# rcanut/nhwcodec

Hardware: AMD Instinct MI355X
Metric: encode Mpixels/s (512x512 RGB batch) (higher is better)
Workload: dtype int16

## Files before the change

nhwcodec_amd/csrc/nhw_tail_wave.h:

```cpp
#include <type_traits>
#ifndef NHW_TAIL_WAVE_H
#define NHW_TAIL_WAVE_H

#include "nhw_tail_dev.h"

namespace nhw {

struct M4 { uint64_t w[4]; };
DEV M4 operator&(M4 a, M4 b) { return M4{ { a.w[0] & b.w[0], a.w[1] & b.w[1], a.w[2] & b.w[2], a.w[3] & b.w[3] } }; }
DEV M4 operator|(M4 a, M4 b) { return M4{ { a.w[0] | b.w[0], a.w[1] | b.w[1], a.w[2] | b.w[2], a.w[3] | b.w[3] } }; }
DEV M4 operator~(M4 a) { return M4{ { ~a.w[0], ~a.w[1], ~a.w[2], ~a.w[3] } }; }
DEV M4 m4_zero() { return M4{ { 0, 0, 0, 0 } }; }
DEV M4 up1(M4 a) { return M4{ { a.w[0] << 1, (a.w[1] << 1) | (a.w[0] >> 63), (a.w[2] << 1) | (a.w[1] >> 63), (a.w[3] << 1) | (a.w[2] >> 63) } }; }
DEV M4 dn1(M4 a) { return M4{ { (a.w[0] >> 1) | (a.w[1] << 63), (a.w[1] >> 1) | (a.w[2] << 63), (a.w[2] >> 1) | (a.w[3] << 63), a.w[3] >> 1 } }; }
DEV M4 dn2(M4 a) { return M4{ { (a.w[0] >> 2) | (a.w[1] << 62), (a.w[1] >> 2) | (a.w[2] << 62), (a.w[2] >> 2) | (a.w[3] << 62), a.w[3] >> 2 } }; }
DEV M4 dn3(M4 a) { return M4{ { (a.w[0] >> 3) | (a.w[1] << 61), (a.w[1] >> 3) | (a.w[2] << 61), (a.w[2] >> 3) | (a.w[3] << 61), a.w[3] >> 3 } }; }
DEV uint64_t low_bits(int n) { return n <= 0 ? 0ull : (n >= 64 ? ~0ull : ((1ull << n) - 1)); }
DEV M4 col_range(int lo, int hi)
{
	M4 r;
	r.w[0] = low_bits(hi + 1) & ~low_bits(lo);
	r.w[1] = low_bits(hi + 1 - 64) & ~low_bits(lo - 64);
	r.w[2] = low_bits(hi + 1 - 128) & ~low_bits(lo - 128);
	r.w[3] = low_bits(hi + 1 - 192) & ~low_bits(lo - 192);
	return r;
}
#define TB(m, k) ((int)__builtin_amdgcn_inverse_ballot_w64((m).w[k]))
#define BALLOT4(m, arr, expr) do { { const int x = arr[0]; (m).w[0] = __ballot(expr); } { const int x = arr[1]; (m).w[1] = __ballot(expr); } \
	{ const int x = arr[2]; (m).w[2] = __ballot(expr); } { const int x = arr[3]; (m).w[3] = __ballot(expr); } } while (0)

template <int N> DEV unsigned bs_up(unsigned b, int lane, unsigned in0 = 0)
{
	const unsigned seam = (((unsigned)__builtin_amdgcn_readlane((int)b, 63) << 1) | in0) & ((1u << N) - 1);
	(void)lane;
	return (unsigned)__builtin_amdgcn_update_dpp((int)seam, (int)b, 0x138 , 0xF, 0xF, false);
}
DEV unsigned bs_dn(unsigned b, int lane)
{
	const unsigned seam = (unsigned)__builtin_amdgcn_readlane((int)b, 0) >> 1;
	(void)lane;
	return (unsigned)__builtin_amdgcn_update_dpp((int)seam, (int)b, 0x130 , 0xF, 0xF, false);
}
#define BS_PREDK(b, arr, k0, expr) do { (b) = 0; for (int k_ = (k0); k_ < 4; k_++) { const int x = (arr)[k_]; (b) |= ((expr) ? 1u : 0u) << k_; } } while (0)
#define BS_PRED(b, arr, n, expr) do { (b) = 0; for (int k_ = 0; k_ < (n); k_++) { const int x = (arr)[k_]; (b) |= ((expr) ? 1u : 0u) << k_; } } while (0)
DEV M4 bs_ballot4(unsigned b) { return M4{ { __ballot(b & 1), __ballot(b & 2), __ballot(b & 4), __ballot(b & 8) } }; }
DEV unsigned bs_from4(M4 m) { unsigned b = 0; for (int k = 0; k < 4; k++) b |= (unsigned)__builtin_amdgcn_inverse_ballot_w64(m.w[k]) << k; return b; }

DEV M4 alt_runs(M4 f)
{
	const uint64_t even = 0x5555555555555555ull;
	const M4 pf = up1(f);
	uint64_t sum[4];
	unsigned carry = 0;
	for (int k = 0; k < 4; k++) {
		const uint64_t se = f.w[k] & ~pf.w[k] & even;
		const uint64_t t = f.w[k] + se;
		const unsigned c1 = t < se;
		sum[k] = t + carry;
		carry = c1 | (sum[k] < t);
	}
	M4 r;
	for (int k = 0; k < 4; k++) {
		const uint64_t re = f.w[k] & ~sum[k];
		r.w[k] = (re & even) | (f.w[k] & ~re & ~even);
	}
	return r;
}

DEV int right_of(const int *v, int k, int nk, int d, int lane)
{
	const int a = __shfl(v[k], (lane + d) & 63);
	const int b = k + 1 < nk ? __shfl(v[k + 1], (lane + d) & 63) : 0;
	return lane + d < 64 ? a : b;
}

DEV int ll2_round(int v) { return (v > 0 && v < 256) ? (v & 0xFFFE) : v; }

DEV void ll2_load_row(const int16_t *p, int r, int lane, int *v, M4 *tag, int q, int part, M4 *starts = nullptr, int ps = W )
{
	if (starts) *starts = m4_zero();
	if (r >= H / 2) { v[0] = v[1] = v[2] = 0; *tag = m4_zero(); return; }
	for (int k = 0; k < 3; k++) v[k] = p[r * ps + lane + 64 * k];
	M4 t = m4_zero();
	if (q > 17) {
		int v4[4] = { v[0], v[1], v[2], 0 };
		M4 o, d3;
		BALLOT4(o, v4, x & 1);
		int far[4];
		for (int k = 0; k < 2; k++) far[k] = right_of(v, k, 3, 3, lane);
		d3.w[0] = __ballot(iabs(v[0] - far[0]) > 1); d3.w[1] = __ballot(iabs(v[1] - far[1]) > 1); d3.w[2] = d3.w[3] = 0;
		const M4 f = o & dn1(o) & dn2(o) & dn3(o) & d3 & col_range(0, H / 2 - 4);
		unsigned __int128 m = ((unsigned __int128)f.w[1] << 64) | f.w[0], tg = 0;
		const unsigned __int128 pat = part ? 5 : 15;
		unsigned __int128 st = 0;
		while (m) {
			const uint64_t lo = (uint64_t)m;
			const int j = lo ? __builtin_ctzll(lo) : 64 + __builtin_ctzll((uint64_t)(m >> 64));
			tg |= pat << j; st |= (unsigned __int128)1 << j;
			m &= ~((unsigned __int128)15 << j);
		}
		t.w[0] = (uint64_t)tg; t.w[1] = (uint64_t)(tg >> 64);
		if (starts) { starts->w[0] = (uint64_t)st; starts->w[1] = (uint64_t)(st >> 64); }
	}
	*tag = t;
}

DEV void wave_ll2_verbatim(Ctx *c, int lane)
{
	if (c->defer_verbatim) return;
	__threadfence_block();
	const int nm = c->m->ll_mem_len;
	for (int i = lane; i < nm; i += 64) {
		const int idx = c->ll_mem[i], pos = ((idx >> 7) << 9) + (idx & 127);
		c->jpeg[pos] = c->proc[pos];
	}
}

DEV void wave_ll2(Ctx *c, int part, int lane, bool keep_p, const int16_t *src, int ss )
{
	int16_t *p = c->proc, *jp = c->jpeg;
	const int q = c->q;
	int v0[3], v1[3], v2[3], v3[3];
	M4 t0, t1, t2, t3;
	ll2_load_row(src, 0, lane, v0, &t0, q, part, nullptr, ss);
	ll2_load_row(src, 1, lane, v1, &t1, q, part, nullptr, ss);
	ll2_load_row(src, 2, lane, v2, &t2, q, part, nullptr, ss);
	ll2_load_row(src, 3, lane, v3, &t3, q, part, nullptr, ss);
	const M4 ll = col_range(0, H / 2 - 1);
	for (int r = 0; r < H / 2; r++) {
		int vn[3]; M4 tn;
		ll2_load_row(src, r + 4, lane, vn, &tn, q, part, nullptr, ss);
		if (q > 17) {
			int a0[4] = { v0[0], v0[1], v0[2], 0 }, a1[4] = { v1[0], v1[1], v1[2], 0 }, a2[4] = { v2[0], v2[1], 0, 0 }, a3[4] = { v3[0], v3[1], 0, 0 };
			M4 o, o1, o2, o3, d2;
			BALLOT4(o, a0, x & 1); BALLOT4(o1, a1, x & 1); BALLOT4(o2, a2, x & 1); BALLOT4(o3, a3, x & 1);
			const int f0 = right_of(v0, 0, 3, 2, lane), f1 = right_of(v0, 1, 3, 2, lane);
			d2.w[0] = __ballot(iabs(v0[0] - f0) > 1); d2.w[1] = __ballot(iabs(v0[1] - f1) > 1); d2.w[2] = d2.w[3] = 0;
			d2 = d2 | dn2(t0);
			const M4 cond1 = o & dn1(o) & col_range(1, H / 2 - 1);
			const M4 hbr = cond1 & dn2(o) & col_range(0, H / 2 - 3);
			const M4 skip = part ? up1(t0) : m4_zero();
			const M4 act = ll & ~t0 & ~skip;
			const M4 fired = alt_runs(hbr & d2 & act);
			const M4 bumped = up1(fired);
			M4 vf = m4_zero();
			if (r <= H / 2 - 2) vf = cond1 & ~hbr & o1 & dn1(o1) & ~dn2(o1);
			if (r >= 1 && r <= H / 2 - 4) vf = vf | (~cond1 & o & o1 & dn1(o1) & o2 & ~o3);
			vf = vf & act & ~bumped & ~t1;
			for (int k = 0; k < 2; k++) { v0[k] += TB(bumped, k); v1[k] += TB(vf, k); }
		}
		for (int k = 0; k < 2; k++) {
			const int at = r * W + lane + 64 * k;
			if (keep_p || !part) p[at] = (int16_t)v0[k];
			jp[at] = (int16_t)(TB(t0, k) ? v0[k] : ll2_round(v0[k]));
		}
		for (int k = 0; k < 3; k++) { v0[k] = v1[k]; v1[k] = v2[k]; v2[k] = v3[k]; v3[k] = vn[k]; }
		t0 = t1; t1 = t2; t2 = t3; t3 = tn;
	}
	if (!part) wave_ll2_verbatim(c, lane);
	__threadfence_block();
}

DEV void wave_emit_ll2(Ctx *c, int lane, bool sim)
{
	int16_t *p = c->proc, *jp = c->jpeg;
	const int q = c->q;
	int v0[3], v1[3], v2[3], v3[3];
	M4 t0, t1, t2, t3, s0, s1, s2, s3;
	ll2_load_row(p, 0, lane, v0, &t0, q, 0, &s0);
	ll2_load_row(p, 1, lane, v1, &t1, q, 0, &s1);
	ll2_load_row(p, 2, lane, v2, &t2, q, 0, &s2);
	ll2_load_row(p, 3, lane, v3, &t3, q, 0, &s3);
	const M4 ll = col_range(0, H / 2 - 1);
	int n4 = 0, e = 0, carry = 0;
	for (int r = 0; r < H / 2; r++) {
		int vn[3]; M4 tn, sn;
		ll2_load_row(p, r + 4, lane, vn, &tn, q, 0, &sn);
		if (q > 17) {
			int a0[4] = { v0[0], v0[1], v0[2], 0 }, a1[4] = { v1[0], v1[1], v1[2], 0 }, a2[4] = { v2[0], v2[1], 0, 0 }, a3[4] = { v3[0], v3[1], 0, 0 };
			M4 o, o1, o2, o3, d2;
			BALLOT4(o, a0, x & 1); BALLOT4(o1, a1, x & 1); BALLOT4(o2, a2, x & 1); BALLOT4(o3, a3, x & 1);
			const int f0 = right_of(v0, 0, 3, 2, lane), f1 = right_of(v0, 1, 3, 2, lane);
			d2.w[0] = __ballot(iabs(v0[0] - f0) > 1); d2.w[1] = __ballot(iabs(v0[1] - f1) > 1); d2.w[2] = d2.w[3] = 0;
			d2 = d2 | dn2(t0);
			const M4 cond1 = o & dn1(o) & col_range(1, H / 2 - 1);
			const M4 hbr = cond1 & dn2(o) & col_range(0, H / 2 - 3);
			const M4 act = ll & ~t0;
			const M4 bumped = up1(alt_runs(hbr & d2 & act));
			M4 vf = m4_zero();
			if (r <= H / 2 - 2) vf = cond1 & ~hbr & o1 & dn1(o1) & ~dn2(o1);
			if (r >= 1 && r <= H / 2 - 4) vf = vf | (~cond1 & o & o1 & dn1(o1) & o2 & ~o3);
			vf = vf & act & ~bumped & ~t1;
			for (int k = 0; k < 2; k++) v1[k] += TB(vf, k);
			for (int k = 0; k < 2; k++) v0[k] += TB(bumped, k);
		}
		uint64_t x[2], g[2];
		int byte[2];
		for (int k = 0; k < 2; k++) {
			const int s = v0[k];
			x[k] = __ballot(s > 255 || s < 0);
			byte[k] = s > 255 ? 255 : (s < 0 ? 0 : s);
		}
		if (r == 0) x[0] &= ~1ull;
		g[0] = ~x[0]; g[1] = ~x[1];
		for (int k = 0; k < 2; k++) {
			const int col = lane + 64 * k, a = r * (H / 2) + col;
			const bool exc = (x[k] >> lane) & 1;
			const uint64_t hi = k ? (g[1] & low_bits(lane)) : 0, lo = k ? g[0] : (g[0] & low_bits(lane));
			const int src = hi ? 64 + 63 - __builtin_clzll(hi) : (lo ? 63 - __builtin_clzll(lo) : -1);
			const int b0 = __shfl(byte[0], src & 63), b1 = __shfl(byte[1], src & 63);
			const int prev = src < 0 ? carry : (((src >> 6) ? b1 : b0) & 254);
			if (exc) {
				const int s = v0[k], mag = s > 255 ? s - 255 : -s;
				const int rank = __popcll(x[0] & (k ? ~0ull : low_bits(lane))) + (k ? __popcll(x[1] & low_bits(lane)) : 0);
				uint8_t *ex = c->exw + e + 3 * rank;
				ex[0] = (uint8_t)r; ex[1] = (uint8_t)(col + (s > 255 ? 128 : 0)); ex[2] = (uint8_t)(mag > 255 ? 255 : mag);
				c->ll_bytes[a] = (uint8_t)prev; c->ll_full[a] = (uint8_t)prev;
			} else { c->ll_full[a] = (uint8_t)byte[k]; c->ll_bytes[a] = (uint8_t)(byte[k] & 254); }
			p[r * W + col] = (int16_t)(sim ? v0[k] : 0);
			if (sim) jp[r * W + col] = (int16_t)(TB(t0, k) ? v0[k] : ll2_round(v0[k]));
		}
		e += 3 * (__popcll(x[0]) + __popcll(x[1]));
		if (g[1]) carry = __shfl(byte[1], 63 - __builtin_clzll(g[1])) & 254;
		else if (g[0]) carry = __shfl(byte[0], 63 - __builtin_clzll(g[0])) & 254;
		if (q > 17) {
			const int cnt = __popcll(s0.w[0]) + __popcll(s0.w[1]);
			if (!cnt) { if (lane == 0) c->res4[n4] = 128; n4++; }
			else {
				for (int k = 0; k < 2; k++)
					if ((s0.w[k] >> lane) & 1) {
						const int rank = __popcll(s0.w[0] & (k ? ~0ull : low_bits(lane))) + (k ? __popcll(s0.w[1] & low_bits(lane)) : 0);
						c->res4[n4 + rank] = (uint8_t)(lane + 64 * k + 1 + (rank == cnt - 1 ? 128 : 0));
					}
				n4 += cnt;
			}
		}
		for (int k = 0; k < 3; k++) { v0[k] = v1[k]; v1[k] = v2[k]; v2[k] = v3[k]; v3[k] = vn[k]; }
		t0 = t1; t1 = t2; t2 = t3; t3 = tn;
		s0 = s1; s1 = s2; s2 = s3; s3 = sn;
	}
	if (lane == 0) { c->m->res4_len = q > 17 ? n4 : 0; c->m->exw_len = e; }
}

DEV void det_load_row(const int16_t *p, int r, int lane, int *v, int ps = W)
{
	if (r >= H) { v[0] = v[1] = v[2] = v[3] = 0; return; }
	const bool top = r < H / 2;
	v[0] = top ? 0 : p[r * ps + lane];
	v[1] = top ? 0 : p[r * ps + lane + 64];
	v[2] = p[r * ps + lane + 128];
	v[3] = p[r * ps + lane + 192];
}

DEV unsigned bs_range(int lo, int hi, int lane)
{
	unsigned b = 0;
	for (int k = 0; k < 4; k++) { const int col = lane + 64 * k; b |= (col >= lo && col <= hi ? 1u : 0u) << k; }
	return b;
}

#define DQ_LIM 512
#define DQ_MARK0 (2 * DQ_LIM + 1)
#define DQ_WORDS (DQ_MARK0 + 126)
enum : unsigned { DQ_E8 = 1u << 16, DQ_E7 = 1u << 17, DQ_EM7 = 1u << 18, DQ_DC = 1u << 19, DQ_AC = 1u << 20, DQ_BIG = 1u << 21, DQ_CODE = 1u << 22, DQ_K2 = 1u << 23, DQ_K1 = 1u << 24, DQ_PRP = 1u << 25, DQ_PRN = 1u << 26 };
DEV int dq_index(int x)
{
	const int d = x - 15300;
	const int cl = x < -DQ_LIM ? -DQ_LIM : x > DQ_LIM ? DQ_LIM : x;
	return ((unsigned)d <= 500u && !(d & 3)) ? DQ_MARK0 + (d >> 2) : cl + DQ_LIM;
}
DEV unsigned dq_entry(int i)
{
	if (i >= DQ_MARK0) {
		const int d = 4 * (i - DQ_MARK0);
		if (d % 100) return DQ_BIG;
		const int x = 15300 + d;
		const int v = (x == 15300 || x == 15500) ? 5 : (x == 15400 || x == 15600) ? -5 : x == 15700 ? 6 : -6;
		return (unsigned)(uint16_t)(int16_t)v | DQ_CODE | (x <= 15400 ? DQ_K2 : DQ_K1) | (x == 15700 ? DQ_PRP : 0u) | (x == 15800 ? DQ_PRN : 0u);
	}
	const int x = i - DQ_LIM;
	if (x >= DQ_LIM || x <= -DQ_LIM) return DQ_BIG;
	int a = x;
	if (a < 0) { a = -a; if ((a & 7) < 7) a &= 0xFFF8; a = -a; }
	unsigned e = (unsigned)(uint16_t)(int16_t)dequant_value(a);
	if (x == 8) e |= DQ_E8;
	if (x == 7) e |= DQ_E7;
	if (x == -7) e |= DQ_EM7;
	if (x > 12 && (x & 7) >= 6) e |= DQ_DC;
	if (x < -12 && ((-x) & 7) == 6) e |= DQ_AC;
	return e;
}
template <bool HAND>
DEV void wave_dequant_details(Ctx *c, int part, int lane, const uint32_t *lut , bool keep_p, const int16_t *src, int ss , int16_t *hand = nullptr)
{
	int16_t *p = c->proc, *jp = c->jpeg;
	const bool hq = c->q > 16;
	int cur[4], nxt[4], pend_v[4] = { 0, 0, 0, 0 };
	unsigned pend = 0;
	int q0[4], q1[4], q2[4];
	det_load_row(src, 0, lane, cur, ss);
	det_load_row(src, 1, lane, nxt, ss);
	det_load_row(src, 2, lane, q0, ss); det_load_row(src, 3, lane, q1, ss); det_load_row(src, 4, lane, q2, ss);
#define UP(b) bs_up<4>((b), lane)
#define DN(b) bs_dn((b), lane)
#define BIT(b, k) (((b) >> (k)) & 1u)
	auto row_step = [&](auto k0c, const int r) {
		constexpr int K0 = decltype(k0c)::value;
		int far[4];
		det_load_row(src, r + 5, lane, far, ss);
		const bool top = r < H / 2;
		const int col0 = top ? H / 2 : 0;
		int jv[4] = { pend_v[0], pend_v[1], pend_v[2], pend_v[3] };
		unsigned je = pend;
		int hv[HAND ? 4 : 1];
		if constexpr (HAND) {
			const unsigned above = pend | DN(pend);
			for (int k = K0; k < 4; k++) hv[k] = BIT(above, k) ? 10100 : cur[k];
		}
		pend = 0;
		if (hq && r < H - 1) {
			unsigned P, N, PN, NN;
			BS_PREDK(P, cur, K0, x > 3 && x < 8); BS_PREDK(N, cur, K0, x < -3 && x > -8);
// ... 144 lines not shown
				if (BIT(vnc, k)) {
					int a = cur[k];
					if (a < 0) { a = -a; if (hq ? (a & 7) < 7 : !BIT(keep_low, k)) a &= 0xFFF8; a = -a; }
					jv[k] = dequant_value(a);
				}
			}
			je |= part_p | part_n | (vis & ~wr);
		}
		for (int k = K0; k < 4; k++) {
			const int at = r * W + lane + 64 * k;
			if (keep_p) p[at] = (int16_t)cur[k];
			if (BIT(je, k)) jp[at] = (int16_t)jv[k];
		}
		for (int k = 0; k < 4; k++) { cur[k] = nxt[k]; nxt[k] = q0[k]; q0[k] = q1[k]; q1[k] = q2[k]; q2[k] = far[k]; }
	};
	for (int r = 0; r < H / 2; r++) row_step(std::integral_constant<int, 2>{}, r);
	for (int r = H / 2; r < H; r++) row_step(std::integral_constant<int, 0>{}, r);
#undef UP
#undef DN
#undef BIT
	__threadfence_block();
}

DEV void wave_shrink(Ctx *c, int lane)
{
	int16_t *jp = c->jpeg;
	const int diag = c->q <= 16 ? 16 : 8;
	int jc[4], jn[4];
	unsigned bp, bc, bn;
	unsigned dp, dn_;
	for (int k = 0; k < 4; k++) { jn[k] = jp[lane + 64 * k]; jc[k] = jp[W + lane + 64 * k]; }
	BS_PRED(bp, jn, 4, iabs(x) >= 8); BS_PRED(dp, jn, 4, iabs(x) >= diag);
	BS_PRED(bc, jc, 4, iabs(x) >= 8);
	unsigned dc_;
	BS_PRED(dc_, jc, 4, iabs(x) >= diag);
	for (int k = 0; k < 4; k++) jn[k] = jp[2 * W + lane + 64 * k];
	BS_PRED(bn, jn, 4, iabs(x) >= 8); BS_PRED(dn_, jn, 4, iabs(x) >= diag);
	const unsigned inner = bs_range(1, H - 2, lane), right = bs_range(H / 2, H - 2, lane);
	int g0[4], g1[4];
	for (int k = 0; k < 4; k++) { g0[k] = jp[3 * W + lane + 64 * k]; g1[k] = jp[4 * W + lane + 64 * k]; }
	for (int r = 1; r < H - 1; r++) {
		int jf[4] = { 0, 0, 0, 0 };
		if (r + 4 < H) for (int k = 0; k < 4; k++) jf[k] = jp[(r + 4) * W + lane + 64 * k];
		const unsigned side = bc | dp | dn_;
		const unsigned near = bs_up<4>(side, lane) | bs_dn(side, lane) | bp | bn;
		const unsigned hit = bc & ~near & (r >= H / 2 ? inner : right);
		for (int k = 0; k < 4; k++)
			if ((hit >> k) & 1u) jp[r * W + lane + 64 * k] = (int16_t)(jc[k] > 0 ? jc[k] - 1 : jc[k] + 1);
		bp = bc; bc = bn; dp = dc_; dc_ = dn_;
		for (int k = 0; k < 4; k++) { jc[k] = jn[k]; jn[k] = g0[k]; g0[k] = g1[k]; g1[k] = jf[k]; }
		BS_PRED(bn, jn, 4, iabs(x) >= 8); BS_PRED(dn_, jn, 4, iabs(x) >= diag);
	}
}

struct M8 { uint64_t w[8]; };
DEV M8 operator&(M8 a, M8 b) { M8 r; for (int k = 0; k < 8; k++) r.w[k] = a.w[k] & b.w[k]; return r; }
DEV M8 operator|(M8 a, M8 b) { M8 r; for (int k = 0; k < 8; k++) r.w[k] = a.w[k] | b.w[k]; return r; }
DEV M8 operator~(M8 a) { M8 r; for (int k = 0; k < 8; k++) r.w[k] = ~a.w[k]; return r; }
DEV M8 up1(M8 a, unsigned in = 0) { M8 r; r.w[0] = (a.w[0] << 1) | in; for (int k = 1; k < 8; k++) r.w[k] = (a.w[k] << 1) | (a.w[k - 1] >> 63); return r; }
DEV M8 dn1(M8 a) { M8 r; for (int k = 0; k < 7; k++) r.w[k] = (a.w[k] >> 1) | (a.w[k + 1] << 63); r.w[7] = a.w[7] >> 1; return r; }
DEV M8 dn2(M8 a) { M8 r; for (int k = 0; k < 7; k++) r.w[k] = (a.w[k] >> 2) | (a.w[k + 1] << 62); r.w[7] = a.w[7] >> 2; return r; }
DEV M8 alt_runs(M8 f)
{
	const uint64_t even = 0x5555555555555555ull;
	const M8 pf = up1(f);
	M8 r;
	unsigned carry = 0;
	for (int k = 0; k < 8; k++) {
		const uint64_t se = f.w[k] & ~pf.w[k] & even;
		const uint64_t t = f.w[k] + se;
		const unsigned c1 = t < se;
		const uint64_t sum = t + carry;
		carry = c1 | (sum < t);
		const uint64_t re = f.w[k] & ~sum;
		r.w[k] = (re & even) | (f.w[k] & ~re & ~even);
	}
	return r;
}
#define BALLOT8(m, arr, expr) do { for (int k_ = 0; k_ < 8; k_++) { const int x = arr[k_]; (m).w[k_] = __ballot(expr); } } while (0)

DEV M8 bs_ballot8(unsigned b) { M8 m; for (int k = 0; k < 8; k++) m.w[k] = __ballot(b & (1u << k)); return m; }
DEV unsigned bs_from8(M8 m) { unsigned b = 0; for (int k = 0; k < 8; k++) b |= (unsigned)__builtin_amdgcn_inverse_ballot_w64(m.w[k]) << k; return b; }
DEV bool mult8_from(int x, int from) { return ((unsigned)(x - from) & 0x80000007u) == 0; }

DEV int left_of_dpp(const int *v, int k, int lane, int edge)
{
	const int seam = k ? __builtin_amdgcn_readlane(v[k - 1], 63) : edge;
	(void)lane;
	return __builtin_amdgcn_update_dpp(seam, v[k], 0x138 , 0xF, 0xF, false);
}
DEV int right_of_dpp(const int *v, int k, int nk, int lane, int edge)
{
	const int seam = k + 1 < nk ? __builtin_amdgcn_readlane(v[k + 1], 0) : edge;
	(void)lane;
	return __builtin_amdgcn_update_dpp(seam, v[k], 0x130 , 0xF, 0xF, false);
}

DEV void quant_load_row(const int16_t *p, int r, int lane, int *v, const int16_t *ll = nullptr, const int16_t *hand = nullptr)
{
	if (hand && r < H) {
		for (int k = 0; k < 4; k++) {
			if (r < H / 2 && k < 2) { const int x = ll ? ll[r * H + lane + 64 * k] : p[r * W + lane + 64 * k]; v[k] = (ll && x <= 8000) ? 0 : x; }
			else v[k] = hand[r * H + lane + 64 * k];
		}
		for (int k = 4; k < 8; k++) v[k] = p[r * W + lane + 64 * k];
		return;
	}
	if (ll && r < H) {
		for (int k = 0; k < 4; k++) { const int x = ll[r * H + lane + 64 * k]; v[k] = (r < H / 2 && k < 2 && x <= 8000) ? 0 : x; }
		for (int k = 4; k < 8; k++) v[k] = p[r * W + lane + 64 * k];
		return;
	}
	for (int k = 0; k < 8; k++) v[k] = r < W ? p[r * W + lane + 64 * k] : 0;
}


#define QROW 516
enum : unsigned { QE_AC = 1u << 8, QE_EQ8 = 1u << 9, QE_DC = 1u << 10, QE_R17 = 1u << 11, QE_M7 = 1u << 12, QE_P7 = 1u << 13, QE_N157 = 1u << 14, QE_BIG = 1u << 15, QE_LOUD = 1u << 16 };
#define QLUT 257
DEV int clamp128(int x) { return x < -128 ? -128 : x > 128 ? 128 : x; }
DEV unsigned quant_entry(int x)
{
	const bool neg = x < 0;
	const int m = neg ? -x : x;
	const int mf = (neg && (m & 7) < 7) ? (m & 504) : m;
	const int v = neg ? -mf : mf;
	unsigned e = (unsigned)(v + 7) < 15u ? 128u : (unsigned)((v + 128) & 248);
	if (x <= -13 && x >= -127 && (m & 7) == 6) e |= QE_AC;
	if (x == 8) e |= QE_EQ8;
	if (x >= 13 && x <= 127 && (x & 7) >= 6) e |= QE_DC;
	if (x >= 1 && x <= 7) e |= QE_R17;
	if (x == -7) e |= QE_M7;
	if (x == 7) e |= QE_P7;
	if (x <= -15 && x >= -127 && (m & 7) == 7) e |= QE_N157;
	if (m > 127) e |= QE_BIG;
	if (m >= 7) e |= QE_LOUD;
	return e;
}
DEV void wave_quantise_luma(Ctx *c, int lane, uint8_t *park , uint32_t *lut , bool write_plane, bool dense, bool ll_from_save,
                            const int16_t *hand = nullptr )
{
	const int16_t *const llsrc = ll_from_save ? c->l2save : nullptr;
	uint64_t *const nzq = c->nzq;
	uint8_t *const vals = c->vals;
	unsigned vtotal = 0;
	for (int i = lane; i < QLUT; i += 64) lut[i] = quant_entry(i - 128);
	__threadfence_block();
	int16_t *p = c->proc;
	uint8_t *stream = c->scan;
	int prev[8], cur[8], nxt[8];
	int q0[8];
	quant_load_row(p, 0, lane, cur, llsrc, hand);
	quant_load_row(p, 1, lane, nxt, llsrc, hand);
	quant_load_row(p, 2, lane, q0, llsrc, hand);
	for (int k = 0; k < 8; k++) prev[k] = 0;
	const bool low = c->q <= 16;
	int q4_turn = 0, q4_carry = 0;
	unsigned last_le0 = 0;
	for (int r = 0; r <= W; r++) {
		int far[8];
		quant_load_row(p, r + 3, lane, far, llsrc, hand);
		if (r < W) {
			if (r < H) {
				const int *c4 = cur + 4;
				unsigned g8;
				BS_PRED(g8, c4, 4, mult8_from(x, 8));
				const unsigned both = g8 & bs_dn(g8, lane) & (lane == 63 ? 0x7u : 0xFu);
				last_le0 = __builtin_amdgcn_readlane(cur[7], 63) <= 0;
				if (__any(both != 0)) {
					unsigned g16, le0;
					BS_PRED(g16, c4, 4, mult8_from(x, 16)); BS_PRED(le0, c4, 4, x <= 0);
					const unsigned ple = bs_up<4>(le0, lane, __builtin_amdgcn_readlane(cur[3], 63) <= 0);
					const unsigned cself = both & g16 & ple;
					const unsigned cnext = both & ((g16 & ~ple) | (g8 & ~g16)) & bs_dn(g16, lane) & bs_dn(bs_dn(le0, lane), lane) & (lane >= 62 ? 0x7u : 0xFu);
					const unsigned hit = __any(cnext != 0) ? bs_from4(up1(alt_runs(bs_ballot4(cnext)))) : 0u;
					const unsigned dec = hit | (cself & ~hit);
					for (int k = 0; k < 4; k++) cur[4 + k] -= (dec >> k) & 1;
				}
			} else {
// ... 236 lines not shown
```

profiles/make_design_table.py:

```python
import json, os, re, sys
ROOT = os.path.dirname(os.path.dirname(os.path.abspath(__file__)))
STATS = os.path.join(ROOT, "profiles", "chroma_tail_kernel_stats_1stream_after.txt")
PMC = os.path.join(ROOT, "profiles", "chroma_tail_pmc_after.json")
BATCHES = 7.0
PH = ["L1", "L2", "L3", "L4A", "C0", "C2", "C3", "C4", "C5", "FINAL", "L4B", "L4C", "L4D", "LLC", "L4C2"]
WV = ["DQ1", "DQ0", "EMIT", "QUANT"]
WHAT = {
    "k_front_image": "a1 + a2 + Y2 + Y3 fused: BGR24 -> Y, 4:2:0 chroma planes out, pre-filter (carry chained in the kernel), both directions of the level-1 analysis, LL copy; a workgroup walks an image (32 rows a band, 512 threads, 78 KB LDS)",
    "k_front_plain": "the same without the pre-filter (q >= 22; q <= 16 and the analysis stage from a luma plane): horizontal pass from registers, 64 rows a band",
    "k_dwt_ana<256>": "level-2 luma analysis of the first closed loop, from ll1, without its transposed plane (whole block in LDS, persistent workgroups); the second loop's only for q <= 12 and the stage checks, level-1 chroma analysis only for q <= 14 and the stage checks",
    "k_chroma_l1q": "level-1 chroma analysis from the 4:2:0 byte plane, a quarter of the 256 x 256 block to a workgroup (four a CU); its coefficients are part of SURVEY's 6 B/pixel",
    "k_dwt_ana<128>": "level-2 chroma analysis (only the tests' stage checks run it)",
    "k_chroma_loops": "both chroma closed loops of a component on one LDS residency of its level-2 block: analysis, simulation 1, synthesis, pre-compensation, analysis (+ cl2save), simulation 2, synthesis (four workgroups a CU)",
    "k_dwt_syn<256>": "level-2 luma synthesis of the second closed loop",
    "k_dwt_syn<128>": "level-2 chroma synthesis (only the tests' stage checks run it)",
    "k_l2_recon": "first closed loop: level-2 synthesis + Y8 (tags -> reconstruction) + Y9 (LL1 pre-compensation) + the second level-2 analysis with Y13's copy on one LDS residency of the block; a batch's form stores l2save and rows 0 .. 127 of the work plane's block",
    "L1": "Y5 tag level-2 details", "L2": "Y8, Y9 as a kernel of their own (only the tests' stage checks run it)", "L3": "Y16 LL2 coder (parse), on a stream of its own beside the second dequantiser simulation",
    "L4A": "Y19-Y23: small runs (wavefront per row), residual classification (one table-driven step for every kind) and coding (column walks on LDS tiles)",
    "L4B": "Y24, Y25 position lists + list packing", "L4C": "Y27 detail clean-up (a wavefront takes 64 consecutive rows, neighbours in registers; Y26 only for q >= 22)", "L4D": "Y31 rewrites, on the symbol LIST (non-zero map + values); leaves map and offsets in stream order",
    "L4C2": "Y29 (q >= 22): band reconstruction, half synthesis, res6 / char_res1 / qsetting3 lists",
    "C0": "chroma: copy", "C2": "chroma: dequantiser simulation 1", "C3": "chroma: tags", "C4": "chroma: dequantiser simulation 2",
    "C5": "chroma: marks (running-index fixed point), LL2 emission, quantiser (wavefront per row); V leaves the merged chroma stream as a list", "LLC": "Z1 chroma LL2 coder", "FINAL": "Z2 packetiser + container",
    "k_l4a": "Y19-Y23 of q >= 17: Y21 small runs (wavefront per row, rows in which nothing fires skipped), Y22 + Y23 as ONE column sweep on registers and class tables (eight workgroups a CU)",
    "k_chroma_tail": "chroma tail of a batch: the rows' shifts (running-index fixed point), LL2 emission, then ONE walk: a wavefront reads each plane row once, marks it in registers and quantises it (rows without a candidate and all-quiet rows skipped); cproc is not written; V leaves the merged chroma stream as a list",
    "k_y31": "Y31 rewrites on the symbol LIST (non-zero map + values), 512 threads an image; leaves map and offsets in stream order",
    "k_final": "Z2 packetiser (the luma part from its symbol list, both books) + container; a kernel of its own at six wavefronts a SIMD",
    "k_pack_chroma": "Z2's chroma part: words and ranked book entries from the chroma symbol list (on the chroma stream in the forked order)",
    "DQ1": "a8 dequantiser simulation, first closed loop (wavefront per image)", "DQ0": "a8 dequantiser simulation, second closed loop",
    "EMIT": "Y14/Y15 LL2 emission", "QUANT": "Y28 luma quantiser + Y30: the symbols leave as a list in stream order (wavefront per image); reads the level-2 block from l2save (Y26)",
}


def label(name):
    m = re.match(r"void k_phase<(\d+)>", name)
    if m:
        return f"`k_phase<{PH[int(m.group(1))]}>`", WHAT.get(PH[int(m.group(1))], "")
    m = re.match(r"void k_wave<(\d+)>", name)
    if m:
        return f"`k_wave<{WV[int(m.group(1))]}>`", WHAT.get(WV[int(m.group(1))], "")
    short = name.replace("void ", "").replace("nhw::", "").split("(")[0]
    base = re.sub(r"<.*", "", short)
    return f"`{short}`", WHAT.get(short, WHAT.get(base, ""))


def table():
    pmc = json.load(open(PMC))
    rows, tot_ms, tot_gb = [], 0.0, 0.0
    for ln in open(STATS):
        m = re.match(r"(.{78})\s+(\d+)\s+([\d.]+)\s+([\d.]+)", ln)
        if not m or "at::" in ln or "rocclr" in ln or "k_synth" in ln:
            continue
        name = m.group(1).strip().split("(")[0]
        calls, total = int(m.group(2)), float(m.group(3))
        key = max((k for k in pmc if len(k.strip()) >= 5 and name.startswith(k.strip())), key=len, default=None)
        rd = wr = None
        if key and "FETCH_SIZE" in pmc[key] and "WRITE_SIZE" in pmc[key]:
            rd = 2 * pmc[key]["FETCH_SIZE"]["per_launch"] * 1024 / 1e9 * calls / BATCHES
            wr = pmc[key]["WRITE_SIZE"]["per_launch"] * 1024 / 1e9 * calls / BATCHES
        rows.append((total / BATCHES, name, calls / BATCHES, rd, wr))
        tot_ms += total / BATCHES; tot_gb += (rd or 0) + (wr or 0)
    out = ["| kernel | passes | launches | ms | HBM read + written, GB | TB/s |", "|---|---|---|---|---|---|"]
    for ms, name, calls, rd, wr in sorted(rows, reverse=True):
        lab, what = label(name)
        gb = f"{rd:.2f} + {wr:.2f}" if rd is not None else "n/a"
        tbs = f"{(rd + wr) / ms:.2f}" if rd is not None and ms else ""
        out.append(f"| {lab} | {what} | {calls:.0f} | {ms:.2f} | {gb} | {tbs} |")
    out.append(f"| **sum (one stream, nothing overlaps)** | | | **{tot_ms:.1f}** | **{tot_gb:.1f}** | |")
    return "\n".join(out)


def main():
    path = os.path.join(ROOT, "DESIGN.md")
    s = open(path).read()
    a, b = s.index("<!-- KERNEL_TABLE_BEGIN -->"), s.index("<!-- KERNEL_TABLE_END -->")
    new = s[:a] + "<!-- KERNEL_TABLE_BEGIN -->\n" + table() + "\n" + s[b:]
    if "--check" in sys.argv:
        sys.exit(0 if new == s else 1)
    open(path, "w").write(new)


if __name__ == "__main__":
    main()
```

Baseline: 66130.

## Keep LL2 row masks as per-lane bit states instead of wave-wide ballot masks

Rewrites the LL2 walk so each row's parity, neighbour-parity and tag bits are stored as a small per-lane bit field built with DPP lane shifts, rather than as 256-bit wave masks rebuilt with many ballots every row. The run detection and the alternating-run bump are computed only when some lane has a candidate (__any gates), and the far-neighbour value is read directly from memory instead of shuffled. This cuts ballot/shuffle and scalar-mask work in the per-row loop of wave_ll2 and wave_emit_ll2. In exchange it adds a stale-state recompute path and seam handling across 64-bit words, which is subtle to keep bit-exact.

```diff
diff --git a/nhwcodec_amd/csrc/nhw_tail_wave.h b/nhwcodec_amd/csrc/nhw_tail_wave.h
--- a/nhwcodec_amd/csrc/nhw_tail_wave.h
+++ b/nhwcodec_amd/csrc/nhw_tail_wave.h
@@ -13,8 +13,6 @@
 DEV M4 m4_zero() { return M4{ { 0, 0, 0, 0 } }; }
 DEV M4 up1(M4 a) { return M4{ { a.w[0] << 1, (a.w[1] << 1) | (a.w[0] >> 63), (a.w[2] << 1) | (a.w[1] >> 63), (a.w[3] << 1) | (a.w[2] >> 63) } }; }
 DEV M4 dn1(M4 a) { return M4{ { (a.w[0] >> 1) | (a.w[1] << 63), (a.w[1] >> 1) | (a.w[2] << 63), (a.w[2] >> 1) | (a.w[3] << 63), a.w[3] >> 1 } }; }
-DEV M4 dn2(M4 a) { return M4{ { (a.w[0] >> 2) | (a.w[1] << 62), (a.w[1] >> 2) | (a.w[2] << 62), (a.w[2] >> 2) | (a.w[3] << 62), a.w[3] >> 2 } }; }
-DEV M4 dn3(M4 a) { return M4{ { (a.w[0] >> 3) | (a.w[1] << 61), (a.w[1] >> 3) | (a.w[2] << 61), (a.w[2] >> 3) | (a.w[3] << 61), a.w[3] >> 3 } }; }
 DEV uint64_t low_bits(int n) { return n <= 0 ? 0ull : (n >= 64 ? ~0ull : ((1ull << n) - 1)); }
 DEV M4 col_range(int lo, int hi)
 {
@@ -40,6 +38,18 @@
 	const unsigned seam = (unsigned)__builtin_amdgcn_readlane((int)b, 0) >> 1;
 	(void)lane;
 	return (unsigned)__builtin_amdgcn_update_dpp((int)seam, (int)b, 0x130 , 0xF, 0xF, false);
+}
+DEV int left_of_dpp(const int *v, int k, int lane, int edge)
+{
+	const int seam = k ? __builtin_amdgcn_readlane(v[k - 1], 63) : edge;
+	(void)lane;
+	return __builtin_amdgcn_update_dpp(seam, v[k], 0x138 , 0xF, 0xF, false);
+}
+DEV int right_of_dpp(const int *v, int k, int nk, int lane, int edge)
+{
+	const int seam = k + 1 < nk ? __builtin_amdgcn_readlane(v[k + 1], 0) : edge;
+	(void)lane;
+	return __builtin_amdgcn_update_dpp(seam, v[k], 0x130 , 0xF, 0xF, false);
 }
 #define BS_PREDK(b, arr, k0, expr) do { (b) = 0; for (int k_ = (k0); k_ < 4; k_++) { const int x = (arr)[k_]; (b) |= ((expr) ? 1u : 0u) << k_; } } while (0)
 #define BS_PRED(b, arr, n, expr) do { (b) = 0; for (int k_ = 0; k_ < (n); k_++) { const int x = (arr)[k_]; (b) |= ((expr) ? 1u : 0u) << k_; } } while (0)
@@ -76,35 +86,125 @@
 
 DEV int ll2_round(int v) { return (v > 0 && v < 256) ? (v & 0xFFFE) : v; }
 
-DEV void ll2_load_row(const int16_t *p, int r, int lane, int *v, M4 *tag, int q, int part, M4 *starts = nullptr, int ps = W )
-{
-	if (starts) *starts = m4_zero();
-	if (r >= H / 2) { v[0] = v[1] = v[2] = 0; *tag = m4_zero(); return; }
-	for (int k = 0; k < 3; k++) v[k] = p[r * ps + lane + 64 * k];
-	M4 t = m4_zero();
-	if (q > 17) {
-		int v4[4] = { v[0], v[1], v[2], 0 };
-		M4 o, d3;
-		BALLOT4(o, v4, x & 1);
-		int far[4];
-		for (int k = 0; k < 2; k++) far[k] = right_of(v, k, 3, 3, lane);
-		d3.w[0] = __ballot(iabs(v[0] - far[0]) > 1); d3.w[1] = __ballot(iabs(v[1] - far[1]) > 1); d3.w[2] = d3.w[3] = 0;
-		const M4 f = o & dn1(o) & dn2(o) & dn3(o) & d3 & col_range(0, H / 2 - 4);
-		unsigned __int128 m = ((unsigned __int128)f.w[1] << 64) | f.w[0], tg = 0;
-		const unsigned __int128 pat = part ? 5 : 15;
-		unsigned __int128 st = 0;
-		while (m) {
-			const uint64_t lo = (uint64_t)m;
-			const int j = lo ? __builtin_ctzll(lo) : 64 + __builtin_ctzll((uint64_t)(m >> 64));
-			tg |= pat << j; st |= (unsigned __int128)1 << j;
-			m &= ~((unsigned __int128)15 << j);
-		}
-		t.w[0] = (uint64_t)tg; t.w[1] = (uint64_t)(tg >> 64);
-		if (starts) { starts->w[0] = (uint64_t)st; starts->w[1] = (uint64_t)(st >> 64); }
-	}
-	*tag = t;
-}
-
+enum : unsigned { L2_O = 0, L2_P1 = 3, L2_P2 = 6, L2_T = 9, L2_S = 11, L2_TU = 13, L2_TD = 15 };
+#define L2F(s, f, n) (((s) >> (f)) & ((1u << (n)) - 1))
+#define IB(w) ((unsigned)__builtin_amdgcn_inverse_ballot_w64(w))
+
+DEV unsigned l2_range(int lo, int hi, int lane)
+{
+	unsigned b = 0;
+	for (int k = 0; k < 3; k++) { const int col = lane + 64 * k; b |= (col >= lo && col <= hi ? 1u : 0u) << k; }
+	return b;
+}
+
+DEV unsigned ll2_row_state(const int *v, const int *far, int lane, int part)
+{
+	const unsigned o = (unsigned)(v[0] & 1) | ((unsigned)(v[1] & 1) << 1) | ((unsigned)(v[2] & 1) << 2);
+	const unsigned p1 = bs_dn(o, lane), p2 = bs_dn(p1, lane), p3 = bs_dn(p2, lane);
+	unsigned s = o | (p1 << L2_P1) | (p2 << L2_P2);
+	const unsigned d3 = (iabs(v[0] - far[0]) > 1 ? 1u : 0u) | (iabs(v[1] - far[1]) > 1 ? 2u : 0u);
+	const unsigned f = o & p1 & p2 & p3 & d3 & l2_range(0, H / 2 - 4, lane);
+	if (__any(f != 0)) {
+		const uint64_t pat = part ? 5 : 15;
+		uint64_t tg[2], st[2], kill = 0, over = 0;
+		for (int k = 0; k < 2; k++) {
+			uint64_t m = __ballot((f >> k) & 1u) & ~kill, t = over, b = 0;
+			kill = over = 0;
+			while (m) {
+				const int j = __builtin_ctzll(m);
+				t |= pat << j; b |= 1ull << j;
+				m &= ~(15ull << j);
+				if (j > 60) { kill = 15ull >> (64 - j); over = pat >> (64 - j); }
+			}
+			tg[k] = t; st[k] = b;
+		}
+		s |= (IB(tg[0]) << L2_T) | (IB(tg[1]) << (L2_T + 1)) | (IB(st[0]) << L2_S) | (IB(st[1]) << (L2_S + 1));
+		s |= (IB((tg[0] >> 2) | (tg[1] << 62)) << L2_TD) | (IB(tg[1] >> 2) << (L2_TD + 1));
+		if (part) s |= (IB(tg[0] << 1) << L2_TU) | (IB((tg[1] << 1) | (tg[0] >> 63)) << (L2_TU + 1));
+	}
+	return s;
+}
+
+DEV void l2_right(const int *v, int *x)
+{
+	const int seam = __builtin_amdgcn_readlane(v[1], 0);
+	x[0] = __builtin_amdgcn_update_dpp(seam, v[0], 0x130 , 0xF, 0xF, false);
+	x[1] = __builtin_amdgcn_update_dpp(seam, v[1], 0x130 , 0xF, 0xF, false);
+}
+
+DEV void alt_runs_next2(uint64_t f0, uint64_t f1, uint64_t *b)
+{
+	const uint64_t even = 0x5555555555555555ull;
+	const uint64_t se0 = f0 & ~(f0 << 1) & even, se1 = f1 & ~((f1 << 1) | (f0 >> 63)) & even;
+	const uint64_t s0 = f0 + se0, t1 = f1 + se1, s1 = t1 + (s0 < se0 ? 1u : 0u);
+	const uint64_t re0 = f0 & ~s0, re1 = f1 & ~s1;
+	const uint64_t r0 = (re0 & even) | (f0 & ~re0 & ~even), r1 = (re1 & even) | (f1 & ~re1 & ~even);
+	b[0] = r0 << 1; b[1] = (r1 << 1) | (r0 >> 63);
+}
+
+struct Ll2Win {
+	int v0[2], v1[2], v2[2], v3[2];
+	unsigned s0, s1, s2, s3;
+	int raw[3], far[2];
+	bool stale;
+	const int16_t *p; int ps; int part; bool walk;
+
+	__device__ void fetch(int r, int lane)
+	{
+		if (r >= H / 2) { raw[0] = raw[1] = raw[2] = far[0] = far[1] = 0; return; }
+		const int16_t *row = p + r * ps + lane;
+		for (int k = 0; k < 3; k++) raw[k] = row[64 * k];
+		if (walk) { far[0] = row[3]; far[1] = row[64 + 3]; }
+		else far[0] = far[1] = 0;
+	}
+	__device__ unsigned make(int lane) const { return walk ? ll2_row_state(raw, far, lane, part) : 0u; }
+	__device__ void start(const int16_t *src, int pitch, int q, int part_, int lane)
+	{
+		p = src; ps = pitch; part = part_; walk = q > 17; stale = false;
+		fetch(0, lane); v0[0] = raw[0]; v0[1] = raw[1]; s0 = make(lane);
+		fetch(1, lane); v1[0] = raw[0]; v1[1] = raw[1]; s1 = make(lane);
+		fetch(2, lane); v2[0] = raw[0]; v2[1] = raw[1]; s2 = make(lane);
+		fetch(3, lane); v3[0] = raw[0]; v3[1] = raw[1]; s3 = make(lane);
+		fetch(4, lane);
+	}
+	__device__ void step(int r, int lane)
+	{
+		if (!walk) return;
+		const unsigned o = L2F(s0, L2_O, 3), t0 = L2F(s0, L2_T, 2);
+		unsigned p1 = L2F(s0, L2_P1, 3), p2 = L2F(s0, L2_P2, 3);
+		if (stale) { p1 = bs_dn(o, lane); p2 = bs_dn(p1, lane); }
+		const unsigned cond1 = o & p1 & l2_range(1, H / 2 - 1, lane);
+		const unsigned hbr = cond1 & p2 & l2_range(0, H / 2 - 3, lane);
+		const unsigned act = 3u & ~t0 & ~L2F(s0, L2_TU, 2);
+		unsigned cand = hbr & act, bumped = 0;
+		if (__any(cand != 0)) {
+			int x1[2], x2[2];
+			l2_right(v0, x1); l2_right(x1, x2);
+			const unsigned d2 = (iabs(v0[0] - x2[0]) > 1 ? 1u : 0u) | (iabs(v0[1] - x2[1]) > 1 ? 2u : 0u) | L2F(s0, L2_TD, 2);
+			cand &= d2;
+			if (__any(cand != 0)) {
+				uint64_t b[2];
+				alt_runs_next2(__ballot(cand & 1u), __ballot(cand & 2u), b);
+				bumped = IB(b[0]) | (IB(b[1]) << 1);
+			}
+		}
+		const unsigned o1 = L2F(s1, L2_O, 3);
+		unsigned vf = 0;
+		if (r <= H / 2 - 2) vf = cond1 & ~hbr & o1 & L2F(s1, L2_P1, 3) & ~L2F(s1, L2_P2, 3);
+		if (r >= 1 && r <= H / 2 - 4) vf |= ~cond1 & o & o1 & L2F(s1, L2_P1, 3) & L2F(s2, L2_O, 3) & ~L2F(s3, L2_O, 3);
+		vf &= act & ~bumped & ~L2F(s1, L2_T, 2);
+		for (int k = 0; k < 2; k++) { v0[k] += (int)((bumped >> k) & 1u); v1[k] += (int)((vf >> k) & 1u); }
+		s1 ^= vf;
+		stale = __any(vf != 0);
+	}
+	__device__ void shift(int r, int lane)
+	{
+		const unsigned sn = make(lane);
+		for (int k = 0; k < 2; k++) { v0[k] = v1[k]; v1[k] = v2[k]; v2[k] = v3[k]; v3[k] = raw[k]; }
+		s0 = s1; s1 = s2; s2 = s3; s3 = sn;
+		fetch(r + 5, lane);
+	}
+};
 DEV void wave_ll2_verbatim(Ctx *c, int lane)
 {
 	if (c->defer_verbatim) return;
@@ -119,43 +219,16 @@
 DEV void wave_ll2(Ctx *c, int part, int lane, bool keep_p, const int16_t *src, int ss )
 {
 	int16_t *p = c->proc, *jp = c->jpeg;
-	const int q = c->q;
-	int v0[3], v1[3], v2[3], v3[3];
-	M4 t0, t1, t2, t3;
-	ll2_load_row(src, 0, lane, v0, &t0, q, part, nullptr, ss);
-	ll2_load_row(src, 1, lane, v1, &t1, q, part, nullptr, ss);
-	ll2_load_row(src, 2, lane, v2, &t2, q, part, nullptr, ss);
-	ll2_load_row(src, 3, lane, v3, &t3, q, part, nullptr, ss);
-	const M4 ll = col_range(0, H / 2 - 1);
+	Ll2Win w;
+	w.start(src, ss, c->q, part, lane);
 	for (int r = 0; r < H / 2; r++) {
-		int vn[3]; M4 tn;
-		ll2_load_row(src, r + 4, lane, vn, &tn, q, part, nullptr, ss);
-		if (q > 17) {
-			int a0[4] = { v0[0], v0[1], v0[2], 0 }, a1[4] = { v1[0], v1[1], v1[2], 0 }, a2[4] = { v2[0], v2[1], 0, 0 }, a3[4] = { v3[0], v3[1], 0, 0 };
-			M4 o, o1, o2, o3, d2;
-			BALLOT4(o, a0, x & 1); BALLOT4(o1, a1, x & 1); BALLOT4(o2, a2, x & 1); BALLOT4(o3, a3, x & 1);
-			const int f0 = right_of(v0, 0, 3, 2, lane), f1 = right_of(v0, 1, 3, 2, lane);
-			d2.w[0] = __ballot(iabs(v0[0] - f0) > 1); d2.w[1] = __ballot(iabs(v0[1] - f1) > 1); d2.w[2] = d2.w[3] = 0;
-			d2 = d2 | dn2(t0);
-			const M4 cond1 = o & dn1(o) & col_range(1, H / 2 - 1);
-			const M4 hbr = cond1 & dn2(o) & col_range(0, H / 2 - 3);
-			const M4 skip = part ? up1(t0) : m4_zero();
-			const M4 act = ll & ~t0 & ~skip;
-			const M4 fired = alt_runs(hbr & d2 & act);
-			const M4 bumped = up1(fired);
-			M4 vf = m4_zero();
-			if (r <= H / 2 - 2) vf = cond1 & ~hbr & o1 & dn1(o1) & ~dn2(o1);
-			if (r >= 1 && r <= H / 2 - 4) vf = vf | (~cond1 & o & o1 & dn1(o1) & o2 & ~o3);
-			vf = vf & act & ~bumped & ~t1;
-			for (int k = 0; k < 2; k++) { v0[k] += TB(bumped, k); v1[k] += TB(vf, k); }
-		}
+		w.step(r, lane);
 		for (int k = 0; k < 2; k++) {
 			const int at = r * W + lane + 64 * k;
-			if (keep_p || !part) p[at] = (int16_t)v0[k];
-			jp[at] = (int16_t)(TB(t0, k) ? v0[k] : ll2_round(v0[k]));
-		}
-		for (int k = 0; k < 3; k++) { v0[k] = v1[k]; v1[k] = v2[k]; v2[k] = v3[k]; v3[k] = vn[k]; }
-		t0 = t1; t1 = t2; t2 = t3; t3 = tn;
+			if (keep_p || !part) p[at] = (int16_t)w.v0[k];
+			jp[at] = (int16_t)(((w.s0 >> (L2_T + k)) & 1u) ? w.v0[k] : ll2_round(w.v0[k]));
+		}
+		w.shift(r, lane);
 	}
 	if (!part) wave_ll2_verbatim(c, lane);
 	__threadfence_block();
@@ -165,35 +238,12 @@
 {
 	int16_t *p = c->proc, *jp = c->jpeg;
 	const int q = c->q;
-	int v0[3], v1[3], v2[3], v3[3];
-	M4 t0, t1, t2, t3, s0, s1, s2, s3;
-	ll2_load_row(p, 0, lane, v0, &t0, q, 0, &s0);
-	ll2_load_row(p, 1, lane, v1, &t1, q, 0, &s1);
-	ll2_load_row(p, 2, lane, v2, &t2, q, 0, &s2);
-	ll2_load_row(p, 3, lane, v3, &t3, q, 0, &s3);
-	const M4 ll = col_range(0, H / 2 - 1);
+	Ll2Win w;
+	w.start(p, W, q, 0, lane);
 	int n4 = 0, e = 0, carry = 0;
 	for (int r = 0; r < H / 2; r++) {
-		int vn[3]; M4 tn, sn;
-		ll2_load_row(p, r + 4, lane, vn, &tn, q, 0, &sn);
-		if (q > 17) {
-			int a0[4] = { v0[0], v0[1], v0[2], 0 }, a1[4] = { v1[0], v1[1], v1[2], 0 }, a2[4] = { v2[0], v2[1], 0, 0 }, a3[4] = { v3[0], v3[1], 0, 0 };
-			M4 o, o1, o2, o3, d2;
-			BALLOT4(o, a0, x & 1); BALLOT4(o1, a1, x & 1); BALLOT4(o2, a2, x & 1); BALLOT4(o3, a3, x & 1);
-			const int f0 = right_of(v0, 0, 3, 2, lane), f1 = right_of(v0, 1, 3, 2, lane);
-			d2.w[0] = __ballot(iabs(v0[0] - f0) > 1); d2.w[1] = __ballot(iabs(v0[1] - f1) > 1); d2.w[2] = d2.w[3] = 0;
-			d2 = d2 | dn2(t0);
-			const M4 cond1 = o & dn1(o) & col_range(1, H / 2 - 1);
-			const M4 hbr = cond1 & dn2(o) & col_range(0, H / 2 - 3);
-			const M4 act = ll & ~t0;
-			const M4 bumped = up1(alt_runs(hbr & d2 & act));
-			M4 vf = m4_zero();
-			if (r <= H / 2 - 2) vf = cond1 & ~hbr & o1 & dn1(o1) & ~dn2(o1);
-			if (r >= 1 && r <= H / 2 - 4) vf = vf | (~cond1 & o & o1 & dn1(o1) & o2 & ~o3);
-			vf = vf & act & ~bumped & ~t1;
-			for (int k = 0; k < 2; k++) v1[k] += TB(vf, k);
-			for (int k = 0; k < 2; k++) v0[k] += TB(bumped, k);
-		}
+		w.step(r, lane);
+		const int *v0 = w.v0;
 		uint64_t x[2], g[2];
 		int byte[2];
 		for (int k = 0; k < 2; k++) {
@@ -218,26 +268,26 @@
 				c->ll_bytes[a] = (uint8_t)prev; c->ll_full[a] = (uint8_t)prev;
 			} else { c->ll_full[a] = (uint8_t)byte[k]; c->ll_bytes[a] = (uint8_t)(byte[k] & 254); }
 			p[r * W + col] = (int16_t)(sim ? v0[k] : 0);
-			if (sim) jp[r * W + col] = (int16_t)(TB(t0, k) ? v0[k] : ll2_round(v0[k]));
+			if (sim) jp[r * W + col] = (int16_t)(((w.s0 >> (L2_T + k)) & 1u) ? v0[k] : ll2_round(v0[k]));
 		}
 		e += 3 * (__popcll(x[0]) + __popcll(x[1]));
 		if (g[1]) carry = __shfl(byte[1], 63 - __builtin_clzll(g[1])) & 254;
 		else if (g[0]) carry = __shfl(byte[0], 63 - __builtin_clzll(g[0])) & 254;
 		if (q > 17) {
-			const int cnt = __popcll(s0.w[0]) + __popcll(s0.w[1]);
-			if (!cnt) { if (lane == 0) c->res4[n4] = 128; n4++; }
+			const unsigned st = L2F(w.s0, L2_S, 2);
+			if (!__any(st != 0)) { if (lane == 0) c->res4[n4] = 128; n4++; }
 			else {
+				const uint64_t sw[2] = { __ballot(st & 1u), __ballot(st & 2u) };
+				const int cnt = __popcll(sw[0]) + __popcll(sw[1]);
 				for (int k = 0; k < 2; k++)
-					if ((s0.w[k] >> lane) & 1) {
-						const int rank = __popcll(s0.w[0] & (k ? ~0ull : low_bits(lane))) + (k ? __popcll(s0.w[1] & low_bits(lane)) : 0);
+					if ((st >> k) & 1u) {
+						const int rank = __popcll(sw[0] & (k ? ~0ull : low_bits(lane))) + (k ? __popcll(sw[1] & low_bits(lane)) : 0);
 						c->res4[n4 + rank] = (uint8_t)(lane + 64 * k + 1 + (rank == cnt - 1 ? 128 : 0));
 					}
 				n4 += cnt;
 			}
 		}
-		for (int k = 0; k < 3; k++) { v0[k] = v1[k]; v1[k] = v2[k]; v2[k] = v3[k]; v3[k] = vn[k]; }
-		t0 = t1; t1 = t2; t2 = t3; t3 = tn;
-		s0 = s1; s1 = s2; s2 = s3; s3 = sn;
+		w.shift(r, lane);
 	}
 	if (lane == 0) { c->m->res4_len = q > 17 ? n4 : 0; c->m->exw_len = e; }
 }
@@ -548,19 +598,6 @@
 DEV M8 bs_ballot8(unsigned b) { M8 m; for (int k = 0; k < 8; k++) m.w[k] = __ballot(b & (1u << k)); return m; }
 DEV unsigned bs_from8(M8 m) { unsigned b = 0; for (int k = 0; k < 8; k++) b |= (unsigned)__builtin_amdgcn_inverse_ballot_w64(m.w[k]) << k; return b; }
 DEV bool mult8_from(int x, int from) { return ((unsigned)(x - from) & 0x80000007u) == 0; }
-
-DEV int left_of_dpp(const int *v, int k, int lane, int edge)
-{
-	const int seam = k ? __builtin_amdgcn_readlane(v[k - 1], 63) : edge;
-	(void)lane;
-	return __builtin_amdgcn_update_dpp(seam, v[k], 0x138 , 0xF, 0xF, false);
-}
-DEV int right_of_dpp(const int *v, int k, int nk, int lane, int edge)
-{
-	const int seam = k + 1 < nk ? __builtin_amdgcn_readlane(v[k + 1], 0) : edge;
-	(void)lane;
-	return __builtin_amdgcn_update_dpp(seam, v[k], 0x130 , 0xF, 0xF, false);
-}
 
 DEV void quant_load_row(const int16_t *p, int r, int lane, int *v, const int16_t *ll = nullptr, const int16_t *hand = nullptr)
 {
diff --git a/profiles/make_design_table.py b/profiles/make_design_table.py
--- a/profiles/make_design_table.py
+++ b/profiles/make_design_table.py
@@ -1,6 +1,6 @@
 import json, os, re, sys
 ROOT = os.path.dirname(os.path.dirname(os.path.abspath(__file__)))
-STATS = os.path.join(ROOT, "profiles", "chroma_tail_kernel_stats_1stream_after.txt")
+STATS = os.path.join(ROOT, "profiles", "ll2_lanes_kernel_stats_1stream_after.txt")
 PMC = os.path.join(ROOT, "profiles", "chroma_tail_pmc_after.json")
 BATCHES = 7.0
 PH = ["L1", "L2", "L3", "L4A", "C0", "C2", "C3", "C4", "C5", "FINAL", "L4B", "L4C", "L4D", "LLC", "L4C2"]
```

Result: no change. 67350 (median of 3 runs) (+1.8%).
